# brson/synth2

Hardware: AMD Instinct MI355X
Metric: voice-samples/sec (mono) at 64k voices per GPU, 48 kHz, 1024-frame buffers (higher is better)
Workload: dtype f32

## Files before the change

include/s2r.h:

```cpp
#ifndef S2R_H
#define S2R_H
#include <stddef.h>
#include <stdint.h>

#ifdef __cplusplus
extern "C" {
#endif

#define S2R_ABI_VERSION 4

typedef enum {
    S2R_OK = 0,
    S2R_ERR_INVALID = -1,
    S2R_ERR_NO_DEVICE = -2,
    S2R_ERR_HIP = -3,
    S2R_ERR_PATCH_SYNTAX = -4,
    S2R_ERR_PATCH_RANGE = -5,
    S2R_ERR_TOO_MANY_FRAMES = -6,
    S2R_ERR_OFFSET_OVERFLOW = -7,
    S2R_ERR_OUT_OF_MEMORY = -8
} s2r_status;

typedef enum { S2R_OSC_SQUARE = 0, S2R_OSC_SAW = 1, S2R_OSC_TRIANGLE = 2, S2R_OSC_SINE = 3,
               S2R_OSC_DPW_SAW = 4, S2R_OSC_DPW_SQUARE = 5, S2R_OSC_DPW_TRIANGLE = 6 } s2r_osc_kind;
// ... 183 lines not shown

typedef void (*s2r_voice_log_fn)(void *user, uint32_t voice_index, uint8_t note);
int s2r_set_voice_log(s2r_synth *s, s2r_voice_log_fn fn, void *user);

uint32_t s2r_abi_version(void);
const char *s2r_build_id(void);
uint32_t s2r_shard_voices(const s2r_synth *s);
uint32_t s2r_block_voices(const s2r_synth *s);
uint32_t s2r_device_count(const s2r_synth *s);
uint64_t s2r_double_release_count(const s2r_synth *s);
int s2r_set_low_latency(s2r_synth *s, int enabled);
int s2r_low_latency_active(const s2r_synth *s);
#define S2R_EXCHANGE_HANDLE_BYTES 64
int s2r_exchange_create(s2r_synth *s, uint32_t n_ranks, void *handle_out, size_t handle_bytes);
int s2r_exchange_attach(s2r_synth *s, uint32_t rank, uint32_t n_ranks, const void *handle, size_t handle_bytes);
int s2r_set_resident(s2r_synth *s, int enabled);
int s2r_resident_active(const s2r_synth *s);
int s2r_quiesce(s2r_synth *s);
int s2r_set_timing(s2r_synth *s, int enabled);
int s2r_set_flat_shortcut(s2r_synth *s, int enabled);
int s2r_set_coeff_stream(s2r_synth *s, int enabled);
int s2r_set_uniform_window(s2r_synth *s, int enabled);
int s2r_uniform_window_chunks(s2r_synth *s, uint64_t *chunks);
float s2r_last_render_ms(s2r_synth *s);
const char *s2r_last_error(const s2r_synth *s);
const char *s2r_status_string(int status);


#define S2R_STREAM_CHARS_PER_SAMPLE 18u
#define S2R_STREAM_FRAMES 4096u
#define S2R_STREAM_RATE_HZ 32000u
size_t s2r_stream_frame_json(const float *samples, size_t n, char *out, size_t cap);

int s2r_parse_patch_text(const char *text, size_t len, s2r_patch *out, char *err_buf, size_t err_cap);

float s2r_voice_pan(float pan, float key_spread, uint8_t note);
void s2r_pan_gains(float p, float *gl, float *gr);

float s2r_voice_gain(float level, float velocity_sens, float velocity);

void s2r_fader_gains(float pan, float w, float fader, float pan_shift, float *gl, float *gr);

float s2r_send_gain(float g, float send);

typedef struct s2r_voice_pool s2r_voice_pool;
s2r_voice_pool *s2r_voice_pool_create(uint32_t total_voices);
// ... 14 lines not shown
```

synth2_amd/csrc/s2r_host.cpp:

```cpp
#include <hip/hip_runtime.h>
#include <algorithm>
#include <cmath>
#include <cstdarg>
#include <cstdio>
#include <cstdlib>
#include <cstring>
#include <ctime>
#include <atomic>
#include <memory>
#include <new>
#include <string>
#include <vector>

#include "s2r.h"
#include "s2r_device.h"
#include "s2r_math.h"
#include "s2r_patch.h"
#include "s2r_post.h"
#include "s2r_rules.h"
#include "s2r_voices.h"

namespace {

constexpr int kEventSlots = 4;
// ... 1828 lines not shown
            CREATE_HIP(hipMalloc((void **)&s->partials2[1], (size_t)s->n_blocks * partials_stride(cfg->max_frames) * sizeof(float)));
            CREATE_HIP(hipMalloc((void **)&s->heads2[1], pv * sizeof(int32_t)));
            CREATE_HIP(hipMemsetAsync(s->heads2[1], 0xff, pv * sizeof(int32_t), s->stream));
            CREATE_HIP(hipMalloc((void **)&s->tevcopy2[1], (size_t)s->tev_capacity * sizeof(S2rTimedEvent)));
            CREATE_HIP(hipMalloc((void **)&s->ov_words, sizeof(S2rOverlapWords)));
            CREATE_HIP(hipMemsetAsync(s->ov_words, 0, sizeof(S2rOverlapWords), s->stream));
            s->ov_enabled = true;
        }
    }
    CREATE_HIP(hipEventCreate(&s->t0));
    CREATE_HIP(hipEventCreate(&s->t1));
    {
        float table[1024];
        build_sin_table(table);
        if (crc32_bytes(table, sizeof table) != kSinTableCrc) {
            fprintf(stderr, "libs2r: regenerated SIN_TABLE does not match the reference table (CRC mismatch)\n");
            release_all(s);
            return S2R_ERR_INVALID;
        }
        CREATE_HIP(hipMalloc((void **)&s->sin_dev, sizeof table));
        CREATE_HIP(hipMemcpy(s->sin_dev, table, sizeof table, hipMemcpyHostToDevice));
        CREATE_HIP(hipMalloc((void **)&s->noise_dev, 65536 * sizeof(float)));
        CREATE_HIP(s2r_launch_noise_table(s->noise_dev, s->stream));
        CREATE_HIP(hipMalloc((void **)&s->uw_count_dev, sizeof(uint32_t)));
        CREATE_HIP(hipMemsetAsync(s->uw_count_dev, 0, sizeof(uint32_t), s->stream));
    }
    CREATE_HIP(hipStreamSynchronize(s->stream));
#undef CREATE_HIP
    *out = s;
    return S2R_OK;
}


int s2r_create(const s2r_config *cfg, s2r_synth **out) {
    if (!cfg || !out || cfg->struct_size != sizeof(s2r_config)) return S2R_ERR_INVALID;
    *out = nullptr;
    if (cfg->n_devices <= 1) {
        s2r_config one = *cfg;
        if (cfg->n_devices == 1) one.device = cfg->devices[0];
        one.n_devices = 0;
        return create_single(&one, nullptr, nullptr, out);
    }
    const uint32_t n = cfg->n_devices;
    const uint32_t bv = cfg->block_voices ? cfg->block_voices : 256u;
    if (n > S2R_MAX_DEVICES || cfg->total_voices == 0 || cfg->max_frames == 0 || cfg->reserved0 != 0) return S2R_ERR_INVALID;
    if (cfg->shard_begin || cfg->shard_voices || cfg->shard_index || cfg->shard_count > 1 || cfg->mix_groups > 1) return S2R_ERR_INVALID;
    if (bv < 64 || bv > 1024 || (bv & 63u) || cfg->total_voices % ((uint64_t)n * bv)) return S2R_ERR_INVALID;
    if (cfg->shard_interleave && ((cfg->shard_interleave & 15u) || bv % cfg->shard_interleave)) return S2R_ERR_INVALID;
// ... 1030 lines not shown
}

uint32_t s2r_shard_voices(const s2r_synth *s) { return s ? s->shard_voices : 0; }
uint32_t s2r_block_voices(const s2r_synth *s) { return s ? s->block_voices : 0; }
uint32_t s2r_device_count(const s2r_synth *s) { return s ? (s->kids.empty() ? 1u : (uint32_t)s->kids.size()) : 0; }
uint64_t s2r_double_release_count(const s2r_synth *s) { return s ? s->double_release : 0; }

int s2r_set_flat_shortcut(s2r_synth *s, int enabled) {
    if (!s) return S2R_ERR_INVALID;
    S2R_QUIESCE(s);
    s->no_flat_shortcut = enabled == 0;
    for (s2r_synth *kid : s->kids) kid->no_flat_shortcut = s->no_flat_shortcut;
    return S2R_OK;
}

int s2r_set_uniform_window(s2r_synth *s, int enabled) {
    if (!s) return S2R_ERR_INVALID;
    S2R_QUIESCE(s);
    s->uniform_window = enabled != 0;
    for (s2r_synth *kid : s->kids) kid->uniform_window = s->uniform_window;
    return S2R_OK;
}

int s2r_uniform_window_chunks(s2r_synth *s, uint64_t *chunks) {
    if (!s || !chunks) return S2R_ERR_INVALID;
    S2R_QUIESCE(s);
    uint64_t total = 0;
    auto one = [&](s2r_synth *h) -> int {
        if (!h->uw_count_dev) return S2R_OK;
        uint32_t n = 0;
        S2R_HIP(s, hipSetDevice(h->device));
        S2R_HIP(s, hipDeviceSynchronize());
        S2R_HIP(s, hipMemcpy(&n, h->uw_count_dev, sizeof n, hipMemcpyDeviceToHost));
        total += n;
        return S2R_OK;
    };
    if (s->kids.empty()) { S2R_TRY(one(s)); }
    else for (s2r_synth *kid : s->kids) { S2R_TRY(one(kid)); }
    *chunks = total;
    return S2R_OK;
}

int s2r_set_coeff_stream(s2r_synth *s, int enabled) {
    if (!s) return S2R_ERR_INVALID;
    S2R_QUIESCE(s);
    s->use_tab = enabled != 0;
    s->use_arg_events = enabled != 2 && enabled != 4;
    s->bank_dirty = true;
    for (s2r_synth *kid : s->kids) { kid->use_tab = s->use_tab; kid->use_arg_events = s->use_arg_events; kid->bank_dirty = true; }
    return S2R_OK;
}

int s2r_set_low_latency(s2r_synth *s, int enabled) {
    if (!s) return S2R_ERR_INVALID;
    if (s->parent || !s->kids.empty()) return set_err(s, S2R_ERR_INVALID, "s2r_set_low_latency takes a single-device handle");
    S2R_QUIESCE(s);
    if (enabled && !s->res_host) {
        S2R_HIP(s, hipSetDevice(s->device));
        S2R_HIP(s, hipHostMalloc((void **)&s->res_host, 64 * sizeof(uint32_t), kHostPolled));
        std::memset(s->res_host, 0, 64 * sizeof(uint32_t));
        S2R_HIP(s, hipHostGetDevicePointer((void **)&s->res_dev, s->res_host, 0));
        s->res_cmd = s->res_host; s->res_cmd_dev = s->res_dev; s->res_cmd_vram = false;
        S2R_HIP(s, hipHostMalloc((void **)&s->res_gran, S2R_RES_GRANULE_FRAMES * sizeof(unsigned long long), kHostPolled));
        std::memset(s->res_gran, 0, S2R_RES_GRANULE_FRAMES * sizeof(unsigned long long));
// ... 204 lines not shown
```

synth2_amd/csrc/s2r_kern_common.h:

```cpp
#pragma once
#include <hip/hip_runtime.h>
#include <type_traits>
#include "s2r_device.h"
#include "s2r_math.h"

namespace {

__constant__ uint64_t c_exp2f_table[S2R_EXP2F_N] = S2R_EXP2F_TABLE_INIT;

constexpr int kChunk = 16;
constexpr uint32_t kSuperMax = 256;
constexpr uint32_t kSuperWhole = 1024;
constexpr int kP = 4;
constexpr uint32_t kTileRow = 68;

typedef float f4 __attribute__((ext_vector_type(4)));
typedef int i4 __attribute__((ext_vector_type(4)));
typedef unsigned u4 __attribute__((ext_vector_type(4)));
typedef unsigned short us4 __attribute__((ext_vector_type(4)));
typedef double d4 __attribute__((ext_vector_type(4)));
typedef unsigned long long ul4 __attribute__((ext_vector_type(4)));

__device__ __forceinline__ f4 vfma(f4 a, f4 b, f4 c) { return __builtin_elementwise_fma(a, b, c); }
__device__ __forceinline__ d4 vfma(d4 a, d4 b, d4 c) { return __builtin_elementwise_fma(a, b, c); }
// ... 1022 lines not shown
            const uint32_t rs = s_cmd[10] & 1u;
            ctl.mt.out = rs ? pl.rows_mine[1] : pl.rows_mine[0];
            ctl.mt.rows = rs ? pl.rows[1] : pl.rows[0];
            ctl.mt.rows_done = pl.mt.rows_done + rs;
            ctl.mt.rows_target = s_cmd[9];
            ctl.mt.stereo = 0;
            ctl.mt.done = S2rDone{pl.mt.xmode == 2 ? pl.done_flag + sel : nullptr, s_cmd[3], pl.done_counter + sel};
            ctl.mt.final_out = sel == 0u ? pl.final_out[0] : sel == 1u ? pl.final_out[1] : pl.final_out[2];
            ctl.mt.final_done = S2rDone{pl.final_flag + sel, s_cmd[3], nullptr};
            ctl.mt.final_stereo = stereo;
        } else {
            ctl.mt.out = o;
            ctl.mt.stereo = stereo;
            ctl.mt.done = S2rDone{pl.done_flag + sel, s_cmd[3], pl.done_counter + sel};
            if (s_cmd[12] != 0u && pl.granules != nullptr) { ctl.mt.granules = pl.granules; ctl.mt.granule_tag = s_cmd[3]; }
        }
        }
        if (frames != 0u && frames <= a.p.frames) fill(ctl);
        __syncthreads();
    }
    if (blockIdx.x == 0u && tid == 0u) __hip_atomic_store(pl.exited, pl.launch_id, __ATOMIC_RELAXED, __HIP_MEMORY_SCOPE_SYSTEM);
}

template <int OSC, int SRC, int FILT = 0, bool FMV = false, int NZ = 0, bool AFLAT = false, bool UW = false>
__device__ __forceinline__ void chunk_fast(const S2rRenderParams &p, VoiceRegs &r, const EnvRun &ea, const EnvRun &em,
                                           const FlatCache &fc, const OscK &k, uint32_t o_chunk, const float *tab,
                                           const uint64_t *sT, const float *sSin, bool live, uint32_t tile_m0,
                                           float *pv_dst, const FiltCoef *fcoef = nullptr, Filt2 *f2 = nullptr,
                                           const float *win = nullptr) {
    constexpr bool SMALL = NZ >= 1, ALIGNED = NZ == 2;
    static_assert(!UW || (SRC == 1 && FILT == 0 && !FMV && NZ == 2 && !AFLAT), "the uniform window replaces one variant only");
    tile_set_base(tile_m0);
    f4 xq[4], bq[4], gq[4], pq[4], iq[4];
    f4 a0w[4], ampw[4], nzw[4];
    if (UW) {
#pragma unroll
        for (int q = 0; q < 4; ++q) {
            xq[q] = *reinterpret_cast<const f4 *>(win + 4 * q);
            a0w[q] = *reinterpret_cast<const f4 *>(win + S2R_UW_FRAMES + 4 * q);
            ampw[q] = *reinterpret_cast<const f4 *>(win + 2u * S2R_UW_FRAMES + 4 * q);
            nzw[q] = *reinterpret_cast<const f4 *>(win + 3u * S2R_UW_FRAMES + 4 * q);
        }
    } else if (SRC == 1) {
        const uint32_t plane = p.tab.plane;
#pragma unroll
        for (int q = 0; q < 4; ++q) {
            xq[q] = load_f4u(tab + 4 * q);
            if (FILT != 0) { bq[q] = load_f4u(tab + plane + 4 * q); gq[q] = load_f4u(tab + 2u * plane + 4 * q); }
            if (FMV) pq[q] = load_f4u(tab + p.tab.fm_plane * plane + 4 * q);
        }
    }
    const double rcp_period = (OSC == S2R_OSC_SINE && !FMV) ? s2r_rcp_f64(k.period) : 0.0;
    r.last = live ? r.last : 0.0f;
    const float ea_slope = live ? ea.s0 : 0.0f, ea_base = live ? ea.s1 : 0.0f, ea_y0 = live ? ea.s2 : 0.0f;
    const float xc0 = live ? fc.xc : 1.0f;
    f4 amp[4], nz[4];
    const float t_chunk = (float)o_chunk;
    const uint32_t o_lo = o_chunk & 0xffffu;
    uint32_t o01 = pk_add_u16(o_lo | (o_lo << 16), 0x00010000u), o23 = pk_add_u16(o01, 0x00020002u);
    const uint32_t seed_pair = (r.seed_rot & 0xffffu) | (r.seed_rot << 16);
    f4 t_small = splat(t_chunk) + (f4){0.0f, 1.0f, 2.0f, 3.0f};
    f4 nzt[4];
    if (ALIGNED && !UW) {
        const float *np = p.noise_tab + ((r.seed_rot ^ o_chunk) & 0xffffu);
#pragma unroll
        for (int q = 0; q < 4; ++q) nzt[q] = *reinterpret_cast<const f4 *>(np + 4 * q);
    }
#pragma unroll
    for (int q = 0; q < 4; ++q) {
        f4 t;
        if (UW) {
            nz[q] = nzw[q]; amp[q] = ampw[q];
            continue;
        } else if (ALIGNED) {
            t = t_small;
            t_small = t_small + splat(4.0f);
            nz[q] = nzt[q];
        } else if (SMALL) {
            t = t_small;
            nz[q] = hash_noise4_low16(seed_pair, o01, o23);
            t_small = t_small + splat(4.0f);
            o01 = pk_add_u16(o01, 0x00040004u); o23 = pk_add_u16(o23, 0x00040004u);
        } else {
            const u4 ou = (u4)(o_chunk + 4u * q) + (u4){0u, 1u, 2u, 3u};
            t = __builtin_convertvector(ou, f4);
            nz[q] = hash_noise4(r.seed_rot, t) + splat(p.noise_level);
        }
        if (AFLAT) amp[q] = splat(ea_slope * (t_chunk - ea_base) + ea_y0);
        else amp[q] = splat(ea_slope) * pk_add4(t, splat(-ea_base)) + splat(ea_y0);
        if (SRC == 0) xq[q] = splat(xc0);
        if (SRC == 1 && FMV) {
            const f4 f_osc = pq[q] * splat(r.pitch);
            pq[q] = splat(p.sr) / f_osc;
            iq[q] = splat(1.0f) / pq[q];
        }
        if (SRC == 2) {
            const f4 mod = splat(em.s0) * (t - splat(em.s1)) + splat(em.s2);
            const f4 f_lpf = pow2_sleef_core4(mod * splat(p.amt_lpf)) * splat(p.lpf_freq);
            const f4 num = splat(-2.0f * 3.14159274101257324f) * f_lpf;
            const f4 arg = p.fast_div_sr ? div_const_nocheck4(num, p.sr, p.rcp_sr) : (num / splat(p.sr));
// ... 37 lines not shown
        f4 y;
#pragma unroll
        for (int j = 0; j < 4; ++j) {
            if (FILT == 0) {
                y[j] = __builtin_fmaf(a0[j], sv[j], xq[q][j] * r.last);
                r.last = y[j];
            } else {
                FiltCoef cj = *fcoef;
                if (SRC == 1) { cj.alpha = xq[q][j]; cj.beta = bq[q][j]; cj.gamma = gq[q][j]; }
                y[j] = dsp_filter_apply(FILT, cj, sv[j], *f2);
            }
        }
        f4 out = y * amp[q];
        if (FILT != 0) out = (f4)((u4)out & livemask);
        tile_store4(q, out);
        outs[q] = out;
    }
    if (pv_dst) {
#pragma unroll
        for (int q = 0; q < 4; ++q) *reinterpret_cast<f4u *>(pv_dst + 4 * q) = outs[q];
    }
}

__device__ __forceinline__ void uw_fill(const S2rRenderParams &p, const EnvRun &ea, uint32_t seed_rot, uint32_t o_run, uint32_t run,
                                        const float *tab_run, float *win, uint32_t lane) {
    const uint32_t n_quads = 4u * run;
    for (uint32_t q0 = 0; q0 < n_quads; q0 += 64u) {
        const uint32_t Q = q0 + lane;
        if (Q < n_quads) {
            const uint32_t o = o_run + 4u * Q;
            const f4 x = load_f4u(tab_run + 4u * Q);
            const f4 a0 = pk_sub4(splat(1.0f), x);
            const f4 t = splat((float)o) + (f4){0.0f, 1.0f, 2.0f, 3.0f};
            const f4 amp = splat(ea.s0) * pk_add4(t, splat(-ea.s1)) + splat(ea.s2);
            const f4 nz = *reinterpret_cast<const f4 *>(p.noise_tab + ((seed_rot ^ (o & ~15u)) & 0xffffu) + (o & 15u));
            float *w = win + 4u * Q;
            *reinterpret_cast<f4 *>(w) = x;
            *reinterpret_cast<f4 *>(w + S2R_UW_FRAMES) = a0;
            *reinterpret_cast<f4 *>(w + 2u * S2R_UW_FRAMES) = amp;
            *reinterpret_cast<f4 *>(w + 3u * S2R_UW_FRAMES) = nz;
        }
    }
    __builtin_amdgcn_wave_barrier();
}

}
```

synth2_amd/csrc/s2r_render_onepole.inc:

```
#include "s2r_kern_common.h"

namespace {

template <int OSC, bool FM, int MODE, int MAXT, bool UWK = false>
__device__ __forceinline__ void render_fill(const S2rRenderArgs &a, const FillCtl &ctl) {
    const S2rRenderParams &p = a.p;
    constexpr bool PV = MODE == 1;
    constexpr bool TEV = MODE == 2;
    const uint32_t kSuper = p.super_frames;
    __shared__ uint64_t sT[S2R_EXP2F_N];
    __shared__ __attribute__((aligned(8))) float sSin[OSC == S2R_OSC_SINE ? 2048 : 2];
    extern __shared__ __attribute__((aligned(16))) float s_dyn[];
    __shared__ uint32_t s_word;

    const uint32_t tid = threadIdx.x;
    const uint32_t lane = tid & 63u, wave = tid >> 6, n_waves = blockDim.x >> 6;
    constexpr uint32_t VW = 64;
    constexpr uint32_t GW = VW / 16;
    const uint32_t n_groups = n_waves * GW;
    float *const sW = s_dyn;
    constexpr uint32_t kTile = kChunk * kTileRow;
    const uint32_t sw_floats = s2r_sw_buffers(p.frames, kSuper) * n_groups * kSuper;
    float *const tile = s_dyn + sw_floats + wave * kTile;
    float *const wave_scratch = s_dyn + sw_floats + n_waves * kTile + wave * (64u + (UWK ? S2R_UW_PLANES * p.uw_frames : 0u));
    uint32_t uw_chunks = 0;
    const uint32_t tile_lds = (uint32_t)__builtin_amdgcn_readfirstlane((int)(uint32_t)(uintptr_t)tile);
    const uint32_t vi = blockIdx.x * blockDim.x + tid;
#if defined(S2R_STAMPS)
    uint32_t stamp_k = 0;
    auto stamp = [&](uint32_t slot) { if (p.stamps && lane == 0 && slot < 16u) p.stamps[(size_t)(vi >> 6) * 16u + slot] = __builtin_amdgcn_s_memtime(); };
    stamp(0);
#else
    auto stamp = [&](uint32_t) {};
    uint32_t stamp_k = 0; (void)stamp_k;
#endif
    uint32_t dbg_events = 0, dbg_dense = 0, dbg_general = 0, dbg_runs = 0, dbg_runchunks = 0;
    unsigned long long dbg_t_dense = 0, dbg_t_run = 0;
    unsigned long long dbg_t_top = 0, dbg_t_sel = 0; (void)dbg_t_top; (void)dbg_t_sel;
    unsigned long long dbg_t_pick1 = 0, dbg_t_casc = 0; (void)dbg_t_pick1; (void)dbg_t_casc;
    (void)dbg_events; (void)dbg_dense; (void)dbg_general; (void)dbg_runs; (void)dbg_runchunks; (void)dbg_t_dense; (void)dbg_t_run;
#if defined(S2R_STAMPS)
#define S2R_DBG_NOW() __builtin_amdgcn_s_memtime()
#else
#define S2R_DBG_NOW() 0ull
#endif

    tl_mark(p.timeline, p.tl_slot, 0);
    if (tid < S2R_EXP2F_N) sT[tid] = c_exp2f_table[tid];
// ... 60 lines not shown
        ev_frame = 0xffffffffu;
        if (ev_idx >= 0) { ev_next = tev_at(ev_idx); ev_frame = ev_next.frame; }
    }
    bool took_release = false;
    auto take_releases = [&]() {
        while (ev_idx >= 0 && !(ev_next.flags & S2R_EV_RESTART)) {
            const uint32_t rel = r.offset + ev_next.frame;
            const bool base_ok = r.offset <= (1u << 24) || r.offset >= 0u - ctl.frames;
            if (!(base_ok && rel <= (1u << 24))) break;
            if ((ev_next.flags & S2R_EV_RELEASE) && live && !r.released) {
                r.released = true;
                r.release_u = rel;
                took_release = true;
            }
            ev_dirty = true;
            ev_idx = ev_next.next;
            ev_frame = 0xffffffffu;
            if (ev_idx >= 0) { ev_next = tev_at(ev_idx); ev_frame = ev_next.frame; }
        }
    };
    if (TEV) take_releases();
    r.seed_rot = (seed << 5) | (seed >> 27);

    const float rel_f = r.released ? (float)r.release_u : 4294967296.0f;
    r.ro_a = __builtin_fmaxf(rel_f, p.amp.sus_off); r.end_a = r.ro_a + p.amp.R;
    r.ro_m = __builtin_fmaxf(rel_f, p.mod.sus_off); r.end_m = r.ro_m + p.mod.R;

    OscK k_const = make_osck<OSC>(p.sr / (1.0f * r.pitch));
    uint32_t seed_now = seed;

    EnvRun ea = env_stage_at(p.amp, r.ro_a, r.end_a, (float)r.offset);
    EnvRun em = env_stage_at(p.mod, r.ro_m, r.end_m, (float)r.offset);
    float thr_min = __builtin_fminf(ea.s3, em.s3);
    FlatCache fc;
    fc.xc = 0.0f; fc.k = k_const;

    __syncthreads();
    const bool have_tab = p.tab.base != nullptr && !p.no_flat_shortcut;
    FlatConsts fcc = (have_tab && (!FM || p.tab.fm_plane != 0u)) ? flat_consts_from_tables<OSC, FM>(p, r.pitch) : make_flat_consts<OSC, FM>(p, r.pitch, sT);
    fc = refresh_flat<OSC, FM>(fcc, em, fc);

    const bool wave_live = __ballot(live || ev_idx >= 0) != 0ull;
    bool wave_events = TEV && __ballot(ev_idx >= 0) != 0ull;
    const uint32_t x16_frames = ctl.frames & ~(uint32_t)(kChunk - 1);
    const bool fast_ok = __ballot(!(r.phase >= 0.0f && r.phase < 1.0f)) == 0ull &&
        (FM || __ballot(!(k_const.period >= 0x1p-126f && k_const.period < __builtin_inff())) == 0ull);
    const size_t pv_base = (size_t)vi * ctl.frames;
    float *bp = ctl.partials + (size_t)blockIdx.x * p.frames_stride;
    uint32_t buf = 0;

    auto reduce_chunk = [&](uint32_t f_base, uint32_t n_frames) {
        const uint32_t f = lane & 15u, grp = lane >> 4;
        __builtin_amdgcn_wave_barrier();
        if (f < n_frames) {
            const float *src = tile + f * kTileRow + grp * 16u;
            float acc = src[0];
#pragma unroll
            for (int k = 1; k < 16; ++k) acc += src[k];
            sW[(buf * n_groups + wave * GW + grp) * kSuper + f_base + f] = acc;
        }
        __builtin_amdgcn_wave_barrier();
    };

    bool w_flat = false, w_aflat = false, w_aligned = false, w_small = false, w_uni = false;
    auto classify_uniform = [&]() {
        if (!(UWK && !FM) || p.uw_frames == 0u) return;
        const TabCur c = tab_cursor(p.tab, em.s4, r.ro_m > p.mod.sus_off, r.release_u, live);
// ... 58 lines not shown
        } else if (released_now) {
            if (ea.s4 == 2.0f) { const bool rel = t0 < r.end_a;
                ea.s0 = rel ? p.amp.slope_rel : 0.0f; ea.s1 = rel ? r.ro_a : 0.0f; ea.s2 = rel ? p.amp.S : 0.0f;
                ea.s3 = rel ? r.end_a : __builtin_inff(); ea.s4 = rel ? 3.0f : 4.0f; }
            if (em.s4 == 2.0f) { const bool rel = t0 < r.end_m;
                em.s0 = rel ? p.mod.slope_rel : 0.0f; em.s1 = rel ? r.ro_m : 0.0f; em.s2 = rel ? p.mod.S : 0.0f;
                em.s3 = rel ? r.end_m : __builtin_inff(); em.s4 = rel ? 3.0f : 4.0f; }
        }
        else if (took_release) {
            if (ea.s4 == 2.0f) ea.s3 = r.ro_a;
            if (em.s4 == 2.0f) em.s3 = r.ro_m;
        }
        thr_min = __builtin_fminf(ea.s3, em.s3);
        fc = refresh_flat<OSC, FM>(fcc, em, fc);
        return restarted;
    };

    auto apply_events_at = [&](uint32_t fpos) {
        if (!wave_events || __ballot(ev_frame == fpos) == 0ull) return;
        dbg_events += (uint32_t)__builtin_popcountll(__ballot(ev_frame == fpos));
        bool restarted = false;
        if (ev_frame == fpos) restarted = apply_events_lane(fpos);
        if (__ballot(restarted) != 0ull) {
            w_aligned = p.noise_tab != nullptr && __ballot(((r.offset | r.seed_rot) & 15u) != 0u) == 0ull;
            w_small = __ballot(r.offset + ctl.frames > (1u << 24)) == 0ull;
        }
        wave_events = __ballot(ev_idx >= 0) != 0ull;
        w_flat = !p.no_flat_shortcut && __ballot(live && em.s0 != 0.0f) == 0ull &&
                 (!FM || __ballot(!(fc.k.period >= 0x1p-126f && fc.k.period < __builtin_inff())) == 0ull);
        w_aflat = __ballot(live && ea.s0 != 0.0f) == 0ull;
        classify_uniform();
    };

    auto end_of_release = [&](float t0) {
        if (ea.s4 == 3.0f && !(t0 < ea.s3)) { ea.s0 = 0.0f; ea.s1 = 0.0f; ea.s2 = 0.0f; ea.s3 = __builtin_inff(); ea.s4 = 4.0f; }
        if (em.s4 == 3.0f && !(t0 < em.s3)) { em.s0 = 0.0f; em.s1 = 0.0f; em.s2 = 0.0f; em.s3 = __builtin_inff(); em.s4 = 4.0f; }
        if (ea.s4 == 2.0f && !(t0 < ea.s3)) { const bool rel = t0 < r.end_a;
            ea.s0 = rel ? p.amp.slope_rel : 0.0f; ea.s1 = rel ? r.ro_a : 0.0f; ea.s2 = rel ? p.amp.S : 0.0f;
            ea.s3 = rel ? r.end_a : __builtin_inff(); ea.s4 = rel ? 3.0f : 4.0f; }
        if (em.s4 == 2.0f && !(t0 < em.s3)) { const bool rel = t0 < r.end_m;
            em.s0 = rel ? p.mod.slope_rel : 0.0f; em.s1 = rel ? r.ro_m : 0.0f; em.s2 = rel ? p.mod.S : 0.0f;
            em.s3 = rel ? r.end_m : __builtin_inff(); em.s4 = rel ? 3.0f : 4.0f; }
    };

    const uint32_t rf = lane & 15u, rgrp = lane >> 4;
    const float *const tsrc = tile + rf * kTileRow + rgrp * 16u;
// ... 8 lines not shown
#pragma unroll
        for (int q = 1; q < 16; ++q) acc += tv[q];
        return acc;
    };
    auto flush_pending = [&]() {
        *pend_dst = tsum();
        pend_dst = sw_dummy;
        __builtin_amdgcn_wave_barrier();
    };

    bool dense_stay = false;
    for (uint32_t sc0 = 0; sc0 < ctl.frames; sc0 += kSuper) {
        const uint32_t n_sc = (ctl.frames - sc0 < kSuper) ? (ctl.frames - sc0) : kSuper;
        const uint32_t n_x16 = (x16_frames > sc0) ? ((x16_frames - sc0 < n_sc) ? (x16_frames - sc0) : n_sc) : 0u;
        if (wave_live) {
            for (uint32_t c16 = 0; c16 < n_x16; c16 += kChunk) {
                const unsigned long long dbg_tt0 = S2R_DBG_NOW();
                if (TEV) apply_events_at(sc0 + c16);
                const bool dense = TEV && wave_events && fast_ok && have_tab && w_small && w_aligned && p.noise_level == 0.0f &&
                                   (!FM || __ballot(live && !(p.sr >= r.pitch * 0x1p-115f)) == 0ull) &&
                                   (dense_stay || wave_min_u32((ev_frame - (sc0 + c16)) >> 4) <= 2u);
                dbg_t_top += S2R_DBG_NOW() - dbg_tt0;
                if (dense) {
                    bool inside = false;
                    bool idle_exit = false;
                    constexpr uint32_t kNoRel = 0xffffffffu;
                    uint32_t pend_rel = kNoRel;
                    auto commit_plain = [&]() {
                        if (pend_rel != kNoRel) {
                            if ((ev_next.flags & S2R_EV_RELEASE) && live && !r.released) {
                                r.released = true;
                                r.release_u = pend_rel;
                                const float rf = (float)pend_rel;
                                r.ro_a = __builtin_fmaxf(rf, p.amp.sus_off); r.end_a = r.ro_a + p.amp.R;
                                r.ro_m = __builtin_fmaxf(rf, p.mod.sus_off); r.end_m = r.ro_m + p.mod.R;
                            }
                            ev_dirty = true; ev_idx = -1;
                            pend_rel = kNoRel;
                        }
                    };
                    auto plain_now = [&]() { return !(ev_next.flags & S2R_EV_RESTART) && ev_next.next < 0 && ea.s4 <= 1.0f && em.s4 <= 1.0f; };
                    bool plain = plain_now();
                    TabCur cur = tab_cursor(p.tab, em.s4, r.ro_m > p.mod.sus_off, r.release_u, live);
                    const unsigned long long dbg_td0 = S2R_DBG_NOW();
                    while (c16 < n_x16 && wave_events && !idle_exit) {
                        {
// ... 91 lines not shown
                            fc = refresh_flat<OSC, FM>(fcc, em, fc);
                            reclassify_stages();
                        }
                    }
                    const unsigned long long dbg_ts1 = S2R_DBG_NOW();
                    dbg_t_casc += dbg_ts1 - dbg_ts0;
                    uint32_t run = pick_run();
                    dbg_t_pick1 += S2R_DBG_NOW() - dbg_ts1;
                    bool flat = false, tab_ok = false, offs_small = false;
                    if (run) {
                        run = (uint32_t)__builtin_amdgcn_readfirstlane((int)run);
                        offs_small = w_small || __ballot(o_chunk + run * kChunk > (1u << 24)) == 0ull;
                        flat = w_flat;
                        tab_ok = !flat && have_tab && offs_small;
                        if (FM && !flat && !tab_ok) run = 0;
                        if (FM && !flat && __ballot(live && !(p.sr >= r.pitch * 0x1p-115f)) != 0ull) run = 0;
                    }
                    if (run) {
                        ++dbg_runs; dbg_runchunks += run;
                        const unsigned long long dbg_tr0 = S2R_DBG_NOW();
                        dbg_t_sel += dbg_tr0 - dbg_ts0;
                        float *const sw_row = sW + (buf * n_groups + wave * GW + rgrp) * kSuper + rf;
                        const TabCur cur = tab_cursor(p.tab, em.s4, r.ro_m > p.mod.sus_off, r.release_u, live);
                        auto run_chunks = [&](auto src_tag, auto nz_tag, auto aflat_tag, auto uw_tag) {
                            constexpr int SRC = decltype(src_tag)::value;
                            constexpr int NZ = decltype(nz_tag)::value;
                            constexpr bool AFLAT = decltype(aflat_tag)::value;
                            constexpr bool UW = decltype(uw_tag)::value;
                            if (UW) {
                                const uint32_t o_run = (uint32_t)__builtin_amdgcn_readfirstlane((int)o_chunk);
                                uw_fill(p, ea, r.seed_rot, o_run, run, p.tab.base + (ptrdiff_t)(cur.idx + (int32_t)o_chunk), wave_scratch + 64u, lane);
                                uw_chunks += run;
                            }
                            for (uint32_t i = 0; i < run; ++i) {
                                const uint32_t f0 = c16 + i * kChunk;
                                *pend_dst = tsum();
                                float *pvd = (PV && in_range) ? p.per_voice + pv_base + sc0 + f0 : nullptr;
                                const uint32_t oc = o_chunk + i * kChunk;
                                const float *tp = p.tab.base + (ptrdiff_t)(cur.idx + (int32_t)(oc & cur.mask));
                                chunk_fast<OSC, SRC, 0, (FM && SRC == 1), NZ, AFLAT, UW>(p, r, ea, em, fc, FM ? fc.k : k_const, oc, tp, sT, sSin, live,
                                                                              tile_lds, pvd, nullptr, nullptr, wave_scratch + 64u + i * kChunk);
                                __builtin_amdgcn_wave_barrier();
                                pend_dst = sw_row + f0;
                            }
                        };
                        const bool small = p.noise_level == 0.0f && offs_small;
                        const bool aligned = small && w_aligned && ((sc0 + c16) & 15u) == 0u;
                        const bool aflat = aligned && w_aflat;
                        using T = std::true_type; using F = std::false_type;
                        using N0 = std::integral_constant<int, 0>; using N1 = std::integral_constant<int, 1>; using N2 = std::integral_constant<int, 2>;
                        using UWon = std::integral_constant<bool, UWK && !FM>;
                        const bool uw = UWon::value && w_uni && run >= S2R_UW_MIN_RUN;
                        if (tab_ok) {
                            if (aflat) run_chunks(N1{}, N2{}, T{}, F{});
                            else if (aligned && uw) run_chunks(N1{}, N2{}, F{}, UWon{});
                            else if (aligned) run_chunks(N1{}, N2{}, F{}, F{});
                            else if (small) run_chunks(N1{}, N1{}, F{}, F{});
                            else run_chunks(N1{}, N0{}, F{}, F{});
                        } else if (flat) {
                            if (aflat) run_chunks(N0{}, N2{}, T{}, F{});
                            else if (aligned) run_chunks(N0{}, N2{}, F{}, F{});
                            else if (small) run_chunks(N0{}, N1{}, F{}, F{});
                            else run_chunks(N0{}, N0{}, F{}, F{});
                        } else if (!FM) {
                            if (aligned) run_chunks(N2{}, N2{}, F{}, F{});
                            else if (small) run_chunks(N2{}, N1{}, F{}, F{});
                            else run_chunks(N2{}, N0{}, F{}, F{});
                        }
                        c16 += (run - 1u) * kChunk;
                        dbg_t_run += S2R_DBG_NOW() - dbg_tr0;
                        continue;
                    }
                }
                flush_pending();
                ++dbg_general;
                for (uint32_t g = c16; g < c16 + kChunk; g += kP) {
                    FrameCF4 cf; OscK4 kf;
                    closed_form_x4<OSC, FM>(p, r, ea, em, thr_min, fc, fcc, r.offset + sc0 + g, sT, cf, kf);
                    f4 out4;
#pragma unroll
                    for (int j = 0; j < kP; ++j) {
                        FrameCF c1; c1.amp = cf.amp[j]; c1.xc = cf.xc[j]; c1.nz = cf.nz[j];
                        OscK k1 = k_const;
                        if (FM) { k1.period = kf.period[j]; k1.inv_period = kf.inv_period[j];
                                  k1.a = kf.a[j]; k1.b = kf.b[j]; k1.c = kf.c[j]; }
                        const float o = recur_x16<OSC>(p, r, c1, k1, sSin);
                        out4[j] = live ? o : 0.0f;
                    }
                    if (PV) { if (in_range) {
                        float *dst = p.per_voice + pv_base + sc0 + g;
// ... 26 lines not shown
        combine_groups(p, ctl.done, sW + (size_t)buf * n_groups * kSuper, n_groups, kSuper, n_sc, sc0, bp + sc0, tid, blockDim.x, ctl.granules, ctl.granule_tag, ctl.fused || ctl.ov_render_counter != nullptr);
        buf ^= 1u;
        stamp(3u + 2u * stamp_k);
        ++stamp_k;
    }

    if (live) {
        const uint32_t o = r.offset;
        p.v.offset[vi] = (!ev_dirty && o > 0xffffffffu - ctl.frames) ? 0xffffffffu : o + ctl.frames;
        p.v.phase[vi] = r.phase;
        p.v.lpf_last[vi] = r.last;
        if (ev_dirty) {
            p.v.pitch[vi] = r.pitch;
            p.v.release[vi] = r.release_u;
            p.v.flags[vi] = S2R_VF_STARTED | (r.released ? S2R_VF_RELEASED : 0u);
            p.v.seed[vi] = seed_now;
            if (ev_restart) {
                p.v.fx1[vi] = 0.0f; p.v.fx2[vi] = 0.0f; p.v.fy1[vi] = 0.0f; p.v.fy2[vi] = 0.0f;
                p.v.osc_z[vi] = s2r_u2f(S2R_OSC_Z_NONE);
                p.v.program[vi] = program_now;
            }
        }
    }
    if (UWK && uw_chunks != 0u && lane == 0u) __hip_atomic_fetch_add(p.uw_count, uw_chunks, __ATOMIC_RELAXED, __HIP_MEMORY_SCOPE_AGENT);
    if (p.direct_out && ctl.granules == nullptr) signal_done(ctl.done, 1u);
    if (ctl.ov_render_counter != nullptr) ov_signal(ctl.ov_render_counter);
#if defined(S2R_STAMPS)
    if (p.stamps && lane == 0) p.stamps[(size_t)(vi >> 6) * 16u + 8u] = __builtin_amdgcn_s_memrealtime();
    if (ctl.fused) fused_tail(p, ctl, sW, &s_word, p.stamps ? p.stamps + (size_t)(vi >> 6) * 16u : nullptr);
#else
    if (ctl.fused) fused_tail(p, ctl, sW, &s_word);
#endif
#if defined(S2R_STAMPS)
    if (p.stamps && lane == 0) { unsigned long long *d = p.stamps + (size_t)(vi >> 6) * 16u; d[11] = dbg_events; d[12] = (unsigned long long)dbg_dense | ((dbg_t_pick1 & 0x3fffffull) << 20) | ((dbg_t_casc & 0x3fffffull) << 42); d[13] = (dbg_t_top << 32) | (dbg_t_sel & 0xffffffffull); d[14] = dbg_runs;
        d[10] = ((unsigned long long)dbg_runchunks << 48) | ((dbg_t_dense & 0xffffffull) << 24) | (dbg_t_run & 0xffffffull); }
#endif
    stamp(15);
    tl_mark(p.timeline, p.tl_slot, 1);
}

template <int OSC, bool FM, int MODE, int MAXT>
__global__ void __launch_bounds__(MAXT, (MAXT == 256 ? 2 : 1)) s2r_render_kernel(const S2rRenderArgs a) {
    const FillCtl ctl = fill_ctl_from_args(a);
    render_fill<OSC, FM, MODE, MAXT, MAXT == 256>(a, ctl);
}

template <int OSC, bool FM>
// ... 145 lines not shown
```

synth2_amd/synth.py:

```python
import ctypes as C
import os

import numpy as np

from . import build as _build

OSC_SQUARE, OSC_SAW, OSC_TRIANGLE, OSC_SINE = 0, 1, 2, 3
OSC_DPW_SAW, OSC_DPW_SQUARE, OSC_DPW_TRIANGLE = 4, 5, 6

S2R_OK = 0
S2R_ERR_INVALID = -1
S2R_ERR_NO_DEVICE = -2
S2R_ERR_HIP = -3
S2R_ERR_PATCH_SYNTAX = -4
S2R_ERR_PATCH_RANGE = -5
S2R_ERR_TOO_MANY_FRAMES = -6
S2R_ERR_OFFSET_OVERFLOW = -7
S2R_ERR_OUT_OF_MEMORY = -8
MAX_BUSES = 8
MAX_IR_TAPS = 65536
MAX_DELAY_FRAMES = 262144
IR_SEGMENT = 256
METER_BLOCK = 256
LIMITER_MAX_LOOKAHEAD = 1024
# ... 177 lines not shown
        "s2r_sum_partials_device": (C.c_int, [C.c_void_p, C.c_uint32, C.c_size_t, C.c_void_p, C.c_void_p]),
        "s2r_render_voices": (C.c_int, [H, _f32p, C.c_size_t, C.c_uint32]),
        "s2r_process_layers": (C.c_int, [H, C.c_void_p, C.c_uint32, _f32p, C.c_size_t, C.c_uint32]),
        "s2r_set_voice_log": (C.c_int, [H, VOICE_LOG_FN, C.c_void_p]),
        "s2r_export_state": (C.c_int, [H, C.c_void_p]),
        "s2r_import_state": (C.c_int, [H, C.c_void_p]),
        "s2r_set_noise_seed": (C.c_int, [H, C.c_uint32, C.c_uint32]),
        "s2r_shard_voices": (C.c_uint32, [H]),
        "s2r_block_voices": (C.c_uint32, [H]),
        "s2r_device_count": (C.c_uint32, [H]),
        "s2r_double_release_count": (C.c_uint64, [H]),
        "s2r_set_timing": (C.c_int, [H, C.c_int]),
        "s2r_set_low_latency": (C.c_int, [H, C.c_int]),
        "s2r_low_latency_active": (C.c_int, [H]),
        "s2r_set_resident": (C.c_int, [H, C.c_int]),
        "s2r_resident_active": (C.c_int, [H]),
        "s2r_quiesce": (C.c_int, [H]),
        "s2r_exchange_create": (C.c_int, [H, C.c_uint32, C.c_void_p, C.c_size_t]),
        "s2r_exchange_attach": (C.c_int, [H, C.c_uint32, C.c_uint32, C.c_void_p, C.c_size_t]),
        "s2r_set_flat_shortcut": (C.c_int, [H, C.c_int]),
        "s2r_set_coeff_stream": (C.c_int, [H, C.c_int]),
        "s2r_set_uniform_window": (C.c_int, [H, C.c_int]),
        "s2r_uniform_window_chunks": (C.c_int, [H, C.POINTER(C.c_uint64)]),
        "s2r_last_render_ms": (C.c_float, [H]),
        "s2r_last_error": (C.c_char_p, [H]),
        "s2r_parse_patch_text": (C.c_int, [C.c_char_p, C.c_size_t, C.POINTER(Patch), C.c_char_p, C.c_size_t]),
        "s2r_voice_pool_create": (H, [C.c_uint32]),
        "s2r_voice_pool_destroy": (None, [H]),
        "s2r_voice_pool_note_on": (C.c_uint32, [H, C.c_uint8, C.c_float]),
        "s2r_voice_pool_note_off": (C.c_int64, [H, C.c_uint8]),
        "s2r_voice_pool_advance": (None, [H, C.c_uint64]),
        "s2r_voice_pool_next_voice": (C.c_uint32, [H]),
        "s2r_voice_pool_set_threads": (None, [H, C.c_uint32, C.c_size_t]),
        "s2r_voice_pool_resolve": (C.c_uint32, [H, C.c_void_p, C.c_size_t, C.c_uint32, C.c_void_p]),
        "s2r_voice_pool_query": (C.c_int, [H, C.c_uint32, C.POINTER(VoiceState)]),
    }
    for name, (res, args) in sig.items():
        if _build.AB_LIB and not hasattr(L, name):
            continue
        f = getattr(L, name)
        f.restype = res
        f.argtypes = args
    L._fill_raw = C.CFUNCTYPE(C.c_int, H, C.c_void_p, C.c_size_t, C.c_uint32)(("s2r_fill", L))
    _lib = L
    return L

# ... 516 lines not shown

    def import_state(self, arr):
        arr = np.ascontiguousarray(arr, dtype=VOICE_STATE_DTYPE)
        assert arr.size == self.shard_voices
        self._check(self.L.s2r_import_state(self.h, arr.ctypes.data))

    def set_noise_seed(self, voice_index, seed):
        self._check(self.L.s2r_set_noise_seed(self.h, voice_index, seed))

    def set_flat_shortcut(self, enabled=True):
        self._check(self.L.s2r_set_flat_shortcut(self.h, 1 if enabled else 0))

    def set_coeff_stream(self, enabled=True):
        self._check(self.L.s2r_set_coeff_stream(self.h, int(enabled)))

    def set_uniform_window(self, enabled=True):
        self._check(self.L.s2r_set_uniform_window(self.h, 1 if enabled else 0))

    def uniform_window_chunks(self):
        n = C.c_uint64(0)
        self._check(self.L.s2r_uniform_window_chunks(self.h, C.byref(n)))
        return int(n.value)

    def set_low_latency(self, enabled=True):
        self._check(self.L.s2r_set_low_latency(self.h, 1 if enabled else 0))

    @property
    def low_latency_active(self):
        return bool(self.L.s2r_low_latency_active(self.h))

    def set_resident(self, enabled=True):
        self._check(self.L.s2r_set_resident(self.h, 1 if enabled else 0))

    @property
    def resident_active(self):
        return bool(self.L.s2r_resident_active(self.h))

    def quiesce(self):
        self._check(self.L.s2r_quiesce(self.h))

    def exchange_create(self, n_ranks):
        buf = C.create_string_buffer(64)
        self._check(self.L.s2r_exchange_create(self.h, n_ranks, buf, 64))
        return buf.raw

    def exchange_attach(self, rank, n_ranks, handle):
# ... 16 lines not shown
```

Baseline: 1587 billion.

## Stage per-wave noise plane in LDS once per buffer for aligned one-pole chunks

When a wave's live voices share the same offset and seed and the noise level is zero, the kernel loads the whole buffer's noise window from the global noise table once at setup and stores it into the wave's LDS scratch. Aligned one-pole chunks, including the flat-amp and uniform-window variants, then read noise from LDS instead of doing per-chunk global table loads, and uw_fill no longer writes noise. This adds register pressure for the preloaded quads, more template variants, and a second debug counter exposed through a new API. The plane is invalidated on restarts or dense event paths.

```diff
diff --git a/include/s2r.h b/include/s2r.h
--- a/include/s2r.h
+++ b/include/s2r.h
@@ -229,6 +229,7 @@
 int s2r_set_coeff_stream(s2r_synth *s, int enabled);
 int s2r_set_uniform_window(s2r_synth *s, int enabled);
 int s2r_uniform_window_chunks(s2r_synth *s, uint64_t *chunks);
+int s2r_noise_window_chunks(s2r_synth *s, uint64_t *chunks);
 float s2r_last_render_ms(s2r_synth *s);
 const char *s2r_last_error(const s2r_synth *s);
 const char *s2r_status_string(int status);
diff --git a/synth2_amd/csrc/s2r_host.cpp b/synth2_amd/csrc/s2r_host.cpp
--- a/synth2_amd/csrc/s2r_host.cpp
+++ b/synth2_amd/csrc/s2r_host.cpp
@@ -1874,8 +1874,8 @@
         CREATE_HIP(hipMemcpy(s->sin_dev, table, sizeof table, hipMemcpyHostToDevice));
         CREATE_HIP(hipMalloc((void **)&s->noise_dev, 65536 * sizeof(float)));
         CREATE_HIP(s2r_launch_noise_table(s->noise_dev, s->stream));
-        CREATE_HIP(hipMalloc((void **)&s->uw_count_dev, sizeof(uint32_t)));
-        CREATE_HIP(hipMemsetAsync(s->uw_count_dev, 0, sizeof(uint32_t), s->stream));
+        CREATE_HIP(hipMalloc((void **)&s->uw_count_dev, 2 * sizeof(uint32_t)));
+        CREATE_HIP(hipMemsetAsync(s->uw_count_dev, 0, 2 * sizeof(uint32_t), s->stream));
     }
     CREATE_HIP(hipStreamSynchronize(s->stream));
 #undef CREATE_HIP
@@ -2952,7 +2952,7 @@
     return S2R_OK;
 }
 
-int s2r_uniform_window_chunks(s2r_synth *s, uint64_t *chunks) {
+static int window_counter(s2r_synth *s, uint32_t which, uint64_t *chunks) {
     if (!s || !chunks) return S2R_ERR_INVALID;
     S2R_QUIESCE(s);
     uint64_t total = 0;
@@ -2961,7 +2961,7 @@
         uint32_t n = 0;
         S2R_HIP(s, hipSetDevice(h->device));
         S2R_HIP(s, hipDeviceSynchronize());
-        S2R_HIP(s, hipMemcpy(&n, h->uw_count_dev, sizeof n, hipMemcpyDeviceToHost));
+        S2R_HIP(s, hipMemcpy(&n, h->uw_count_dev + which, sizeof n, hipMemcpyDeviceToHost));
         total += n;
         return S2R_OK;
     };
@@ -2970,6 +2970,10 @@
     *chunks = total;
     return S2R_OK;
 }
+
+int s2r_uniform_window_chunks(s2r_synth *s, uint64_t *chunks) { return window_counter(s, 0u, chunks); }
+
+int s2r_noise_window_chunks(s2r_synth *s, uint64_t *chunks) { return window_counter(s, 1u, chunks); }
 
 int s2r_set_coeff_stream(s2r_synth *s, int enabled) {
     if (!s) return S2R_ERR_INVALID;
diff --git a/synth2_amd/csrc/s2r_kern_common.h b/synth2_amd/csrc/s2r_kern_common.h
--- a/synth2_amd/csrc/s2r_kern_common.h
+++ b/synth2_amd/csrc/s2r_kern_common.h
@@ -1068,7 +1068,7 @@
     if (blockIdx.x == 0u && tid == 0u) __hip_atomic_store(pl.exited, pl.launch_id, __ATOMIC_RELAXED, __HIP_MEMORY_SCOPE_SYSTEM);
 }
 
-template <int OSC, int SRC, int FILT = 0, bool FMV = false, int NZ = 0, bool AFLAT = false, bool UW = false>
+template <int OSC, int SRC, int FILT = 0, bool FMV = false, int NZ = 0, bool AFLAT = false, bool UW = false, bool NW = UW>
 __device__ __forceinline__ void chunk_fast(const S2rRenderParams &p, VoiceRegs &r, const EnvRun &ea, const EnvRun &em,
                                            const FlatCache &fc, const OscK &k, uint32_t o_chunk, const float *tab,
                                            const uint64_t *sT, const float *sSin, bool live, uint32_t tile_m0,
@@ -1076,16 +1076,21 @@
                                            const float *win = nullptr) {
     constexpr bool SMALL = NZ >= 1, ALIGNED = NZ == 2;
     static_assert(!UW || (SRC == 1 && FILT == 0 && !FMV && NZ == 2 && !AFLAT), "the uniform window replaces one variant only");
+    static_assert(!NW || (FILT == 0 && NZ == 2), "the noise plane serves aligned one-pole chunks only");
+    static_assert(!UW || NW, "the window's noise is the noise plane");
     tile_set_base(tile_m0);
     f4 xq[4], bq[4], gq[4], pq[4], iq[4];
     f4 a0w[4], ampw[4], nzw[4];
+    if (NW) {
+#pragma unroll
+        for (int q = 0; q < 4; ++q) nzw[q] = *reinterpret_cast<const f4 *>(win + 3u * S2R_UW_FRAMES + 4 * q);
+    }
     if (UW) {
 #pragma unroll
         for (int q = 0; q < 4; ++q) {
             xq[q] = *reinterpret_cast<const f4 *>(win + 4 * q);
             a0w[q] = *reinterpret_cast<const f4 *>(win + S2R_UW_FRAMES + 4 * q);
             ampw[q] = *reinterpret_cast<const f4 *>(win + 2u * S2R_UW_FRAMES + 4 * q);
-            nzw[q] = *reinterpret_cast<const f4 *>(win + 3u * S2R_UW_FRAMES + 4 * q);
         }
     } else if (SRC == 1) {
         const uint32_t plane = p.tab.plane;
@@ -1107,7 +1112,7 @@
     const uint32_t seed_pair = (r.seed_rot & 0xffffu) | (r.seed_rot << 16);
     f4 t_small = splat(t_chunk) + (f4){0.0f, 1.0f, 2.0f, 3.0f};
     f4 nzt[4];
-    if (ALIGNED && !UW) {
+    if (ALIGNED && !NW) {
         const float *np = p.noise_tab + ((r.seed_rot ^ o_chunk) & 0xffffu);
 #pragma unroll
         for (int q = 0; q < 4; ++q) nzt[q] = *reinterpret_cast<const f4 *>(np + 4 * q);
@@ -1121,7 +1126,7 @@
         } else if (ALIGNED) {
             t = t_small;
             t_small = t_small + splat(4.0f);
-            nz[q] = nzt[q];
+            nz[q] = NW ? nzw[q] : nzt[q];
         } else if (SMALL) {
             t = t_small;
             nz[q] = hash_noise4_low16(seed_pair, o01, o23);
@@ -1205,9 +1210,9 @@
     }
 }
 
-__device__ __forceinline__ void uw_fill(const S2rRenderParams &p, const EnvRun &ea, uint32_t seed_rot, uint32_t o_run, uint32_t run,
-                                        const float *tab_run, float *win, uint32_t lane) {
+__device__ __forceinline__ void uw_fill(const EnvRun &ea, uint32_t o_run, uint32_t run, const float *tab_run, float *win, uint32_t lane) {
     const uint32_t n_quads = 4u * run;
+    asm("" : "+v"(lane));
     for (uint32_t q0 = 0; q0 < n_quads; q0 += 64u) {
         const uint32_t Q = q0 + lane;
         if (Q < n_quads) {
@@ -1216,15 +1221,30 @@
             const f4 a0 = pk_sub4(splat(1.0f), x);
             const f4 t = splat((float)o) + (f4){0.0f, 1.0f, 2.0f, 3.0f};
             const f4 amp = splat(ea.s0) * pk_add4(t, splat(-ea.s1)) + splat(ea.s2);
-            const f4 nz = *reinterpret_cast<const f4 *>(p.noise_tab + ((seed_rot ^ (o & ~15u)) & 0xffffu) + (o & 15u));
             float *w = win + 4u * Q;
             *reinterpret_cast<f4 *>(w) = x;
             *reinterpret_cast<f4 *>(w + S2R_UW_FRAMES) = a0;
             *reinterpret_cast<f4 *>(w + 2u * S2R_UW_FRAMES) = amp;
-            *reinterpret_cast<f4 *>(w + 3u * S2R_UW_FRAMES) = nz;
         }
     }
     __builtin_amdgcn_wave_barrier();
 }
 
-}
+struct NwQuads { f4 v[S2R_UW_FRAMES / 256u]; };
+__device__ __forceinline__ NwQuads nw_load(const float *noise_tab, uint32_t seed_rot, uint32_t o_fill, uint32_t lane) {
+    NwQuads n;
+#pragma unroll
+    for (uint32_t i = 0; i < S2R_UW_FRAMES / 256u; ++i) {
+        const uint32_t o = o_fill + 4u * (64u * i + lane);
+        n.v[i] = *reinterpret_cast<const f4 *>(noise_tab + ((seed_rot ^ (o & ~15u)) & 0xffffu) + (o & 15u));
+    }
+    return n;
+}
+__device__ __forceinline__ void nw_store(const NwQuads &n, float *win, uint32_t lane) {
+#pragma unroll
+    for (uint32_t i = 0; i < S2R_UW_FRAMES / 256u; ++i)
+        *reinterpret_cast<f4 *>(win + 3u * S2R_UW_FRAMES + 4u * (64u * i + lane)) = n.v[i];
+    __builtin_amdgcn_wave_barrier();
+}
+
+}
diff --git a/synth2_amd/csrc/s2r_render_onepole.inc b/synth2_amd/csrc/s2r_render_onepole.inc
--- a/synth2_amd/csrc/s2r_render_onepole.inc
+++ b/synth2_amd/csrc/s2r_render_onepole.inc
@@ -24,6 +24,8 @@
     float *const tile = s_dyn + sw_floats + wave * kTile;
     float *const wave_scratch = s_dyn + sw_floats + n_waves * kTile + wave * (64u + (UWK ? S2R_UW_PLANES * p.uw_frames : 0u));
     uint32_t uw_chunks = 0;
+    constexpr uint32_t kNoisePlane = 0x80000000u;
+    auto w_noise = [&]() { return UWK && !FM && (uw_chunks & kNoisePlane) != 0u; };
     const uint32_t tile_lds = (uint32_t)__builtin_amdgcn_readfirstlane((int)(uint32_t)(uintptr_t)tile);
     const uint32_t vi = blockIdx.x * blockDim.x + tid;
 #if defined(S2R_STAMPS)
@@ -130,6 +132,19 @@
     if (TEV) take_releases();
     r.seed_rot = (seed << 5) | (seed >> 27);
 
+    const uint32_t x16_frames = ctl.frames & ~(uint32_t)(kChunk - 1);
+    NwQuads nwq;
+    if (UWK && !FM) {
+        if (p.uw_frames != 0u && p.noise_tab != nullptr && p.noise_level == 0.0f && ctl.frames <= p.uw_frames && x16_frames >= S2R_UW_MIN_RUN * kChunk) {
+            const uint64_t started = __ballot(live);
+            const int first = started != 0ull ? __builtin_ctzll(started) : 0;
+            const uint32_t o_u = (uint32_t)__builtin_amdgcn_readlane((int)r.offset, first), s_u = (uint32_t)__builtin_amdgcn_readlane((int)r.seed_rot, first);
+            const bool odd = ((r.offset | r.seed_rot) & 15u) != 0u || r.offset + ctl.frames > (1u << 24) ||
+                             (live && (r.offset != o_u || r.seed_rot != s_u));
+            if (started != 0ull && __ballot(odd) == 0ull) { uw_chunks = kNoisePlane; nwq = nw_load(p.noise_tab, s_u, o_u, lane); }
+        }
+    }
+
     const float rel_f = r.released ? (float)r.release_u : 4294967296.0f;
     r.ro_a = __builtin_fmaxf(rel_f, p.amp.sus_off); r.end_a = r.ro_a + p.amp.R;
     r.ro_m = __builtin_fmaxf(rel_f, p.mod.sus_off); r.end_m = r.ro_m + p.mod.R;
@@ -147,10 +162,10 @@
     const bool have_tab = p.tab.base != nullptr && !p.no_flat_shortcut;
     FlatConsts fcc = (have_tab && (!FM || p.tab.fm_plane != 0u)) ? flat_consts_from_tables<OSC, FM>(p, r.pitch) : make_flat_consts<OSC, FM>(p, r.pitch, sT);
     fc = refresh_flat<OSC, FM>(fcc, em, fc);
+    if (w_noise()) nw_store(nwq, wave_scratch + 64u, lane);
 
     const bool wave_live = __ballot(live || ev_idx >= 0) != 0ull;
     bool wave_events = TEV && __ballot(ev_idx >= 0) != 0ull;
-    const uint32_t x16_frames = ctl.frames & ~(uint32_t)(kChunk - 1);
     const bool fast_ok = __ballot(!(r.phase >= 0.0f && r.phase < 1.0f)) == 0ull &&
         (FM || __ballot(!(k_const.period >= 0x1p-126f && k_const.period < __builtin_inff())) == 0ull);
     const size_t pv_base = (size_t)vi * ctl.frames;
@@ -255,6 +270,7 @@
         bool restarted = false;
         if (ev_frame == fpos) restarted = apply_events_lane(fpos);
         if (__ballot(restarted) != 0ull) {
+            uw_chunks &= ~kNoisePlane;
             w_aligned = p.noise_tab != nullptr && __ballot(((r.offset | r.seed_rot) & 15u) != 0u) == 0ull;
             w_small = __ballot(r.offset + ctl.frames > (1u << 24)) == 0ull;
         }
@@ -309,6 +325,7 @@
                                    (dense_stay || wave_min_u32((ev_frame - (sc0 + c16)) >> 4) <= 2u);
                 dbg_t_top += S2R_DBG_NOW() - dbg_tt0;
                 if (dense) {
+                    if (UWK && !FM) uw_chunks &= ~kNoisePlane;
                     bool inside = false;
                     bool idle_exit = false;
                     constexpr uint32_t kNoRel = 0xffffffffu;
@@ -446,24 +463,26 @@
                         dbg_t_sel += dbg_tr0 - dbg_ts0;
                         float *const sw_row = sW + (buf * n_groups + wave * GW + rgrp) * kSuper + rf;
                         const TabCur cur = tab_cursor(p.tab, em.s4, r.ro_m > p.mod.sus_off, r.release_u, live);
-                        auto run_chunks = [&](auto src_tag, auto nz_tag, auto aflat_tag, auto uw_tag) {
+                        auto run_chunks = [&](auto src_tag, auto nz_tag, auto aflat_tag, auto uw_tag, auto nw_tag) {
                             constexpr int SRC = decltype(src_tag)::value;
                             constexpr int NZ = decltype(nz_tag)::value;
                             constexpr bool AFLAT = decltype(aflat_tag)::value;
                             constexpr bool UW = decltype(uw_tag)::value;
+                            constexpr bool NW = decltype(nw_tag)::value;
+                            float *const win = wave_scratch + 64u + sc0 + c16;
                             if (UW) {
                                 const uint32_t o_run = (uint32_t)__builtin_amdgcn_readfirstlane((int)o_chunk);
-                                uw_fill(p, ea, r.seed_rot, o_run, run, p.tab.base + (ptrdiff_t)(cur.idx + (int32_t)o_chunk), wave_scratch + 64u, lane);
-                                uw_chunks += run;
+                                uw_fill(ea, o_run, run, p.tab.base + (ptrdiff_t)(cur.idx + (int32_t)o_chunk), win, lane);
                             }
+                            if (NW) uw_chunks += UW ? run * 0x10001u : run << 16;
                             for (uint32_t i = 0; i < run; ++i) {
                                 const uint32_t f0 = c16 + i * kChunk;
                                 *pend_dst = tsum();
                                 float *pvd = (PV && in_range) ? p.per_voice + pv_base + sc0 + f0 : nullptr;
                                 const uint32_t oc = o_chunk + i * kChunk;
                                 const float *tp = p.tab.base + (ptrdiff_t)(cur.idx + (int32_t)(oc & cur.mask));
-                                chunk_fast<OSC, SRC, 0, (FM && SRC == 1), NZ, AFLAT, UW>(p, r, ea, em, fc, FM ? fc.k : k_const, oc, tp, sT, sSin, live,
-                                                                              tile_lds, pvd, nullptr, nullptr, wave_scratch + 64u + i * kChunk);
+                                chunk_fast<OSC, SRC, 0, (FM && SRC == 1), NZ, AFLAT, UW, NW>(p, r, ea, em, fc, FM ? fc.k : k_const, oc, tp, sT, sSin, live,
+                                                                                  tile_lds, pvd, nullptr, nullptr, win + i * kChunk);
                                 __builtin_amdgcn_wave_barrier();
                                 pend_dst = sw_row + f0;
                             }
@@ -474,22 +493,27 @@
                         using T = std::true_type; using F = std::false_type;
                         using N0 = std::integral_constant<int, 0>; using N1 = std::integral_constant<int, 1>; using N2 = std::integral_constant<int, 2>;
                         using UWon = std::integral_constant<bool, UWK && !FM>;
-                        const bool uw = UWon::value && w_uni && run >= S2R_UW_MIN_RUN;
+                        const bool uw = UWon::value && w_uni && w_noise() && run >= S2R_UW_MIN_RUN;
+                        const bool nw = w_noise() && aligned;
                         if (tab_ok) {
-                            if (aflat) run_chunks(N1{}, N2{}, T{}, F{});
-                            else if (aligned && uw) run_chunks(N1{}, N2{}, F{}, UWon{});
-                            else if (aligned) run_chunks(N1{}, N2{}, F{}, F{});
-                            else if (small) run_chunks(N1{}, N1{}, F{}, F{});
-                            else run_chunks(N1{}, N0{}, F{}, F{});
+                            if (aflat && nw) run_chunks(N1{}, N2{}, T{}, F{}, UWon{});
+                            else if (aflat) run_chunks(N1{}, N2{}, T{}, F{}, F{});
+                            else if (aligned && uw) run_chunks(N1{}, N2{}, F{}, UWon{}, UWon{});
+                            else if (nw) run_chunks(N1{}, N2{}, F{}, F{}, UWon{});
+                            else if (aligned) run_chunks(N1{}, N2{}, F{}, F{}, F{});
+                            else if (small) run_chunks(N1{}, N1{}, F{}, F{}, F{});
+                            else run_chunks(N1{}, N0{}, F{}, F{}, F{});
                         } else if (flat) {
-                            if (aflat) run_chunks(N0{}, N2{}, T{}, F{});
-                            else if (aligned) run_chunks(N0{}, N2{}, F{}, F{});
-                            else if (small) run_chunks(N0{}, N1{}, F{}, F{});
-                            else run_chunks(N0{}, N0{}, F{}, F{});
+                            if (aflat && nw) run_chunks(N0{}, N2{}, T{}, F{}, UWon{});
+                            else if (aflat) run_chunks(N0{}, N2{}, T{}, F{}, F{});
+                            else if (nw) run_chunks(N0{}, N2{}, F{}, F{}, UWon{});
+                            else if (aligned) run_chunks(N0{}, N2{}, F{}, F{}, F{});
+                            else if (small) run_chunks(N0{}, N1{}, F{}, F{}, F{});
+                            else run_chunks(N0{}, N0{}, F{}, F{}, F{});
                         } else if (!FM) {
-                            if (aligned) run_chunks(N2{}, N2{}, F{}, F{});
-                            else if (small) run_chunks(N2{}, N1{}, F{}, F{});
-                            else run_chunks(N2{}, N0{}, F{}, F{});
+                            if (aligned) run_chunks(N2{}, N2{}, F{}, F{}, F{});
+                            else if (small) run_chunks(N2{}, N1{}, F{}, F{}, F{});
+                            else run_chunks(N2{}, N0{}, F{}, F{}, F{});
                         }
                         c16 += (run - 1u) * kChunk;
                         dbg_t_run += S2R_DBG_NOW() - dbg_tr0;
@@ -562,7 +586,10 @@
             }
         }
     }
-    if (UWK && uw_chunks != 0u && lane == 0u) __hip_atomic_fetch_add(p.uw_count, uw_chunks, __ATOMIC_RELAXED, __HIP_MEMORY_SCOPE_AGENT);
+    if (UWK && (uw_chunks & ~kNoisePlane) != 0u && lane < 2u) {
+        const uint32_t n = lane == 0u ? (uw_chunks & 0xffffu) : ((uw_chunks & ~kNoisePlane) >> 16);
+        if (n != 0u) __hip_atomic_fetch_add(p.uw_count + lane, n, __ATOMIC_RELAXED, __HIP_MEMORY_SCOPE_AGENT);
+    }
     if (p.direct_out && ctl.granules == nullptr) signal_done(ctl.done, 1u);
     if (ctl.ov_render_counter != nullptr) ov_signal(ctl.ov_render_counter);
 #if defined(S2R_STAMPS)
diff --git a/synth2_amd/synth.py b/synth2_amd/synth.py
--- a/synth2_amd/synth.py
+++ b/synth2_amd/synth.py
@@ -223,6 +223,7 @@
         "s2r_set_coeff_stream": (C.c_int, [H, C.c_int]),
         "s2r_set_uniform_window": (C.c_int, [H, C.c_int]),
         "s2r_uniform_window_chunks": (C.c_int, [H, C.POINTER(C.c_uint64)]),
+        "s2r_noise_window_chunks": (C.c_int, [H, C.POINTER(C.c_uint64)]),
         "s2r_last_render_ms": (C.c_float, [H]),
         "s2r_last_error": (C.c_char_p, [H]),
         "s2r_parse_patch_text": (C.c_int, [C.c_char_p, C.c_size_t, C.POINTER(Patch), C.c_char_p, C.c_size_t]),
@@ -785,6 +786,11 @@
         self._check(self.L.s2r_uniform_window_chunks(self.h, C.byref(n)))
         return int(n.value)
 
+    def noise_window_chunks(self):
+        n = C.c_uint64(0)
+        self._check(self.L.s2r_noise_window_chunks(self.h, C.byref(n)))
+        return int(n.value)
+
     def set_low_latency(self, enabled=True):
         self._check(self.L.s2r_set_low_latency(self.h, 1 if enabled else 0))
 
```

New measurement: 1536 billion. -3.2%, worse.
